# ashawkey/nerf2mesh

Hardware: AMD Instinct MI355X
Metric: train_samples_per_sec (higher is better)
Workload: dtype f32 march/composite, f16 autocast encode+MLP (reference -O recipe); 1 GPU; nerf_synthetic/lego stage-0 -O --bound 1 --dt_gamma 0, 800x800 x 100 synthetic views, num_points target 2^18/GPU (adaptive num_rays), occupancy refresh every 16 steps; diffuse_step=1000, refresh_steps_in_window=64, parallelism=single GPU, occupancy_refresh=single GPU, mlp=fused MFMA field kernels, driver=engine.Stage0Engine (fixed launch sequence), pretrain_steps=1000, params=18367240

## Files before the change

### include/n2m_hip.h

```cpp
#ifndef N2M_HIP_H
#define N2M_HIP_H

#include <stdint.h>

#ifdef __cplusplus
extern "C" {
#endif

#define N2M_ABI_VERSION 1

enum { N2M_F32 = 0, N2M_F16 = 1 };

enum {
    N2M_OK = 0,
    N2M_EINVAL = -1,
    N2M_ENULL = -2,
    N2M_EUNSUPPORTED = -3
};

int n2m_abi_version(void);
const char* n2m_last_error(void);


int n2m_near_far_from_aabb(const float* rays_o, const float* rays_d, const float* aabb, uint32_t N,
// ... 100 lines not shown
                                const int32_t* offsets, void* grad_embeddings, uint32_t B, uint32_t D,
                                uint32_t C, uint32_t L, uint32_t max_level, float S, uint32_t H,
                                uint32_t gridtype, int align_corners, uint32_t interp, int dtype,
                                void* stream);

uint64_t n2m_grid_binned_workspace_bytes(uint32_t B, uint32_t D, uint32_t C, uint32_t max_level,
                                         const int32_t* host_offsets, int dtype, int tv);
int n2m_grid_encode_backward_binned(const void* grad, const float* inputs, const int32_t* host_offsets,
                                    void* grad_embeddings, uint32_t B, uint32_t D, uint32_t C, uint32_t L,
                                    uint32_t max_level, float S, uint32_t H, uint32_t gridtype, int align_corners,
                                    uint32_t interp, int dtype, const float* tv_embeddings, float tv_weight,
                                    float tv_weight_outer, float tv_inner01, const float* tv_scale,
                                    float* found_inf, void* workspace, uint64_t workspace_bytes, void* stream);
int n2m_grad_total_variation_binned(const float* inputs, const float* embeddings, float* grad,
                                    const int32_t* host_offsets, float weight, float weight_outer, float inner01,
                                    const float* weight_scale, uint32_t B, uint32_t D, uint32_t C, uint32_t L, float S,
                                    uint32_t H, uint32_t gridtype, int align_corners, void* workspace,
                                    uint64_t workspace_bytes, void* stream);

int n2m_grid_encode_forward_pair(const float* inputs, const float* embeddings1, const void* embeddings2,
                                 const int32_t* offsets, float* outputs1, void* outputs2, uint32_t B, uint32_t L,
                                 uint32_t max_level, float S, uint32_t H, uint32_t gridtype, int align_corners,
                                 uint32_t interp, float in_scale, float in_offset, void* stream);

int n2m_grid_encode_forward_packed(const float* inputs, const void* packed, const int32_t* offsets, float* outputs1,
                                   void* outputs2, uint32_t B, uint32_t L, uint32_t max_level, float S, uint32_t H,
                                   uint32_t gridtype, int align_corners, uint32_t interp, float in_scale, float in_offset,
                                   void* stream);
int n2m_grid_encode_forward_packed_tv(const float* inputs, const void* packed, const int32_t* offsets, float* outputs1,
                                      void* outputs2, uint32_t B, uint32_t L, uint32_t max_level, float S, uint32_t H,
                                      uint32_t gridtype, int align_corners, uint32_t interp, float in_scale, float in_offset,
                                      float* tv_corners, void* stream);
int n2m_grid_encode_forward_packed_tvterms(const float* inputs, const void* packed, const int32_t* offsets, float* outputs1,
                                           void* outputs2, uint32_t B, uint32_t L, uint32_t max_level, float S, uint32_t H,
                                           uint32_t gridtype, int align_corners, uint32_t interp, float in_scale, float in_offset,
                                           float tv_weight, float tv_weight_outer, float tv_inner01, const float* tv_scale,
                                           float* tv_out, void* stream);
int n2m_grid_backward_tv_corners(const float* tv_corners);

int n2m_grid_encode_forward_packed_levels(const float* inputs, const void* packed, const int32_t* offsets, float* outputs1,
                                          void* outputs2, uint32_t B, uint32_t L, uint32_t max_level, float S, uint32_t H,
                                          uint32_t gridtype, int align_corners, uint32_t interp, float in_scale, float in_offset,
                                          uint32_t level_begin, uint32_t n_levels, void* stream);

uint64_t n2m_grid_binned_pair_workspace_bytes(uint32_t B, uint32_t max_level, const int32_t* host_offsets);
int n2m_grid_encode_backward_binned_pair(const float* grad1, const void* grad2, const float* inputs,
// ... 377 lines not shown
```

### include/n2m_mlp.h

```cpp
#ifndef N2M_MLP_H
#define N2M_MLP_H

#include <stdint.h>

#ifdef __cplusplus
extern "C" {
#endif

int n2m_field_forward(const float* xyz, const float* dirs, const float* h1, const void* h2, const float* w_sigma0,
                      const float* w_sigma1, const float* w_color0, const float* w_color1, const float* w_color2,
                      const float* w_spec0, const float* w_spec1, uint32_t M, int shading, int normalize_dirs, float* sigma, float* rgb,
                      float* specular, void* stream);

int n2m_field_backward(const float* xyz, const float* dirs, const float* h1, const void* h2, const float* w_sigma0,
                       const float* w_sigma1, const float* w_color0, const float* w_color1, const float* w_color2,
                       const float* w_spec0, const float* w_spec1, uint32_t M, int shading, int normalize_dirs, const float* d_sigma,
                       const float* d_rgb, const float* d_specular, float* d_h1, void* d_h2, float* d_w_sigma0,
                       float* d_w_sigma1, float* d_w_color0, float* d_w_color1, float* d_w_color2, float* d_w_spec0,
                       float* d_w_spec1, float* found_inf, void* stream);

int n2m_field_forward_train(const float* xyz, const float* dirs, const float* h1, const void* h2, const float* w_sigma0,
                            const float* w_sigma1, const float* w_color0, const float* w_color1, const float* w_color2,
                            const float* w_spec0, const float* w_spec1, uint32_t M, int shading, int normalize_dirs, float* sigma, float* rgb,
                            float* specular, float* spec_sq_partial, void* stream);
int n2m_field_backward_train(const float* xyz, const float* dirs, const float* h1, const void* h2, const float* w_sigma0,
                             const float* w_sigma1, const float* w_color0, const float* w_color1, const float* w_color2,
                             const float* w_spec0, const float* w_spec1, uint32_t M, int shading, int normalize_dirs, const float* d_sigma,
                             const float* d_rgb, const float* d_specular, float* d_h1, void* d_h2, float* d_w_sigma0,
                             float* d_w_sigma1, float* d_w_color0, float* d_w_color1, float* d_w_color2, float* d_w_spec0,
                             float* d_w_spec1, float* found_inf, float spec_reg, const float* seed, void* stream);
uint32_t n2m_field_spec_partials(void);

#ifdef __cplusplus
}
#endif
// ... 2 lines not shown
```

### nerf2mesh_amd/_lib.py

```python
import ctypes
import os
import threading

_HERE = os.path.dirname(os.path.abspath(__file__))
LIB_PATH = os.environ.get("N2M_HIP_LIB") or os.path.join(_HERE, "lib", "libn2m_hip.so")

_u32, _i32, _f32, _vp, _int, _u64 = ctypes.c_uint32, ctypes.c_int32, ctypes.c_float, ctypes.c_void_p, ctypes.c_int, ctypes.c_uint64

SIGNATURES = {
    "n2m_near_far_from_aabb": [_vp, _vp, _vp, _u32, _f32, _vp, _vp, _vp],
    "n2m_sph_from_ray": [_vp, _vp, _f32, _u32, _vp, _vp],
    "n2m_morton3D": [_vp, _u32, _vp, _vp],
    "n2m_morton3D_invert": [_vp, _u32, _vp, _vp],
    "n2m_packbits": [_vp, _u32, _f32, _vp, _vp],
    "n2m_packbits_dev": [_vp, _u32, _vp, _vp, _vp],
    "n2m_flatten_rays": [_vp, _u32, _u32, _vp, _vp],
    "n2m_march_rays_train": [_vp, _vp, _vp, _f32, _int, _f32, _u32, _u32, _u32, _u32, _vp, _vp, _vp, _vp, _vp, _vp, _vp, _vp, _vp],
    "n2m_march_rays_train_write": [_vp, _vp, _vp, _f32, _int, _f32, _u32, _u32, _u32, _u32, _vp, _vp, _vp, _vp, _vp, _vp, _vp, _u32, _vp],
    "n2m_march_rays_train_fused": [_vp, _vp, _vp, _f32, _int, _f32, _u32, _u32, _u32, _u32, _vp, _vp, _vp, _vp, _vp, _vp, _vp, _vp, _u32, _vp, _u64, _vp],
    "n2m_march_fused_workspace_bytes": [_u32],
    "n2m_march_fallback_count": [_vp],
    "n2m_debug_fill_times": [_int, _vp],
    "n2m_stream_copy": [_vp, _vp, _u64, _u32, _vp],
    "n2m_composite_live_counts": [_vp, _vp],
# ... 5 lines not shown
    "n2m_composite_rays_train_forward": [_vp, _vp, _vp, _vp, _u32, _u32, _f32, _int, _vp, _vp, _vp, _vp, _vp],
    "n2m_composite_rays_train_backward": [_vp, _vp, _vp, _vp, _vp, _vp, _vp, _vp, _vp, _vp, _vp, _u32, _u32, _f32, _int, _vp, _vp, _vp],
    "n2m_composite_loss_train": [_vp, _vp, _vp, _vp, _u32, _u32, _f32, _vp, _vp, _f32, _f32, _f32, _vp, _vp, _vp, _vp, _vp, _vp, _vp, _vp, _vp, _vp],
    "n2m_composite_loss_train_ent": [_vp, _vp, _vp, _vp, _u32, _u32, _f32, _vp, _vp, _f32, _f32, _f32, _vp, _vp, _vp, _vp, _vp, _vp, _vp, _vp, _vp, _f32, _vp],
    "n2m_composite_loss_train_depth": [_vp, _vp, _vp, _vp, _u32, _u32, _f32, _vp, _vp, _f32, _f32, _f32, _vp, _vp, _vp, _vp, _vp, _vp, _vp, _vp, _vp, _f32,
                                       _vp, _vp, _vp, _f32, _int, _vp],
    "n2m_composite_loss_train_ex": [_vp, _vp, _vp, _vp, _u32, _u32, _f32, _vp, _vp, _f32, _f32, _f32, _vp, _vp, _vp, _vp, _vp, _vp, _vp, _vp, _vp, _f32, _int, _vp],
    "n2m_march_rays": [_u32, _u32, _vp, _vp, _vp, _vp, _f32, _int, _f32, _u32, _u32, _u32, _vp, _vp, _vp, _vp, _vp, _vp, _vp, _vp],
    "n2m_composite_rays": [_u32, _u32, _f32, _int, _vp, _vp, _vp, _vp, _vp, _vp, _vp, _vp, _vp],
    "n2m_compact_alive": [_vp, _u32, _vp, _vp, _vp],
    "n2m_select_positive": [_vp, _u32, _u32, _vp, _vp, _vp],
    "n2m_march_rays_dev": [_vp, _u32, _u32, _vp, _vp, _vp, _vp, _f32, _int, _f32, _u32, _u32, _u32, _vp, _vp, _vp, _vp, _vp, _vp, _vp],
    "n2m_composite_rays_dev": [_vp, _u32, _u32, _u32, _f32, _int, _vp, _vp, _vp, _vp, _vp, _vp, _vp, _vp, _vp],
    "n2m_compact_alive_dev": [_vp, _vp, _u32, _u32, _u32, _vp, _vp, _vp],
    "n2m_grid_encode_forward": [_vp, _vp, _vp, _vp, _u32, _u32, _u32, _u32, _u32, _f32, _u32, _vp, _u32, _int, _u32, _int, _vp],
    "n2m_grid_encode_backward": [_vp, _vp, _vp, _vp, _vp, _u32, _u32, _u32, _u32, _u32, _f32, _u32, _vp, _vp, _u32, _int, _u32, _int, _vp],
    "n2m_grad_total_variation": [_vp, _vp, _vp, _vp, _f32, _u32, _u32, _u32, _u32, _f32, _u32, _u32, _int, _int, _vp],
    "n2m_grid_encode_forward_bm": [_vp, _vp, _vp, _vp, _u32, _u32, _u32, _u32, _u32, _f32, _u32, _u32, _int, _u32, _int, _vp],
    "n2m_grid_encode_backward_bm": [_vp, _vp, _vp, _vp, _vp, _u32, _u32, _u32, _u32, _u32, _f32, _u32, _u32, _int, _u32, _int, _vp],
    "n2m_grid_binned_workspace_bytes": [_u32, _u32, _u32, _u32, _vp, _int, _int],
    "n2m_grid_encode_backward_binned": [_vp, _vp, _vp, _vp, _u32, _u32, _u32, _u32, _u32, _f32, _u32, _u32, _int, _u32, _int,
                                        _vp, _f32, _f32, _f32, _vp, _vp, _vp, _u64, _vp],
    "n2m_grid_encode_forward_pair": [_vp, _vp, _vp, _vp, _vp, _vp, _u32, _u32, _u32, _f32, _u32, _u32, _int, _u32, _f32, _f32, _vp],
    "n2m_grid_encode_forward_packed": [_vp, _vp, _vp, _vp, _vp, _u32, _u32, _u32, _f32, _u32, _u32, _int, _u32, _f32, _f32, _vp],
    "n2m_grid_encode_forward_packed_tv": [_vp, _vp, _vp, _vp, _vp, _u32, _u32, _u32, _f32, _u32, _u32, _int, _u32, _f32, _f32, _vp, _vp],
    "n2m_grid_encode_forward_packed_tvterms": [_vp, _vp, _vp, _vp, _vp, _u32, _u32, _u32, _f32, _u32, _u32, _int, _u32, _f32, _f32, _f32, _f32, _f32, _vp, _vp, _vp],
    "n2m_grid_backward_tv_corners": [_vp],
    "n2m_grid_encode_forward_packed_levels": [_vp, _vp, _vp, _vp, _vp, _u32, _u32, _u32, _f32, _u32, _u32, _int, _u32, _f32, _f32, _u32, _u32, _vp],
    "n2m_grid_binned_pair_workspace_bytes": [_u32, _u32, _vp],
    "n2m_grid_encode_backward_binned_pair": [_vp, _vp, _vp, _vp, _vp, _vp, _u32, _u32, _u32, _f32, _u32, _u32, _int, _u32,
                                             _vp, _f32, _f32, _f32, _vp, _vp, _f32, _f32, _int, _vp, _u64, _vp],
    "n2m_grid_encode_backward_binned_pair_half": [_vp, _vp, _vp, _vp, _vp, _vp, _u32, _u32, _u32, _f32, _u32, _u32, _int, _u32,
                                                  _vp, _f32, _f32, _f32, _vp, _vp, _f32, _f32, _int, _vp, _u64, _vp, _int],
    "n2m_sdf_fold_plan": [_vp, _u32, _f32, _f32, _u32, _u32, _f32, _u32, _int, _vp, _vp, _vp, _u32, _vp, _u32, _vp],
    "n2m_sdf_fold_gather": [_vp, _u32, _u32, _vp, _vp, _u32, _vp, _u32, _vp, _vp],
    "n2m_grid_encode_backward_binned_lists": [_vp, _vp, _u32, _vp, _vp, _u32, _u32, _u32, _f32, _u32, _u32, _int, _u32, _vp, _int, _vp, _u64, _vp],
    "n2m_grid_encode_backward_binned_pair_fold": [_vp, _vp, _vp, _vp, _vp, _vp, _u32, _u32, _u32, _f32, _u32, _u32, _int, _u32,
                                                  _vp, _f32, _f32, _f32, _vp, _vp, _f32, _f32, _int, _vp, _u64, _vp, _vp, _f32, _f32, _vp],
    "n2m_occupancy_update_partials": [_u32],
    "n2m_occupancy_points": [_vp, _vp, _vp, _f32, _f32, _vp, _u32, _vp],
    "n2m_occupancy_update": [_vp, _vp, _f32, _u32, _f32, _vp, _vp, _vp, _vp, _vp],
    "n2m_grid_pair_fuse_plan": [_u32, _u32, _vp, ctypes.POINTER(ctypes.c_uint32), ctypes.POINTER(ctypes.c_uint32)],
    "n2m_grid_encode_backward_binned_pair_adam": [_vp, _vp, _vp, _vp, _vp, _vp, _u32, _u32, _u32, _f32, _u32, _u32, _int, _u32,
                                                  _vp, _f32, _f32, _f32, _vp, _vp, _f32, _f32, _vp, _u64, _vp, _vp],
    "n2m_adam_fuse_restore": [_vp, _vp, _u32, _vp, _vp],
    "n2m_grid_tv_terms": [_vp, _vp, _vp, _u32, _u32, _f32, _u32, _u32, _int, _u32, _f32, _f32, _f32, _vp, _f32, _f32, _vp, _vp],
# ... 63 lines not shown
    "n2m_capture_view": [_vp, _u32, _u32, _u32, _u32, _u32, _f32, _f32, _f32, _f32, _vp, _vp, _vp, _vp, _vp, _vp, _u32, _vp],
    "n2m_capture_box_downscale": [_vp, _u32, _u32, _u32, _u32, _vp, _vp],
    "n2m_adam_step": [_vp, ctypes.c_double, ctypes.c_double, _f32, _vp, _vp, _vp, _vp],
    "n2m_adam_step_scaler": [_vp, ctypes.c_double, ctypes.c_double, _f32, _vp, _vp, _vp, _vp, _vp],
    "n2m_ema_update": [_vp, _f32, _vp],
    "n2m_scaler_update": [_vp, _vp, _vp, _vp, _vp, ctypes.c_double, ctypes.c_double, _f32, _f32, _f32, _vp],
    "n2m_scaler_update_slots": [_vp, _vp, _vp, _vp, _vp, _u32, ctypes.c_double, ctypes.c_double, _f32, _f32, _f32, _vp],
    "n2m_scaler_update_slots_loss": [_vp, _vp, _vp, _vp, _vp, _u32, ctypes.c_double, ctypes.c_double, _f32, _f32, _f32, _vp, _u32, _u32, _vp, _vp, _vp],
    "n2m_scaler_update_slots_loss2": [_vp, _vp, _vp, _vp, _vp, _u32, ctypes.c_double, ctypes.c_double, _f32, _f32, _f32, _vp, _u32, _u32, _vp, _vp,
                                      _vp, _u32, _f32, _vp],
    "n2m_scaler_update_slots_loss3": [_vp, _vp, _vp, _vp, _vp, _u32, ctypes.c_double, ctypes.c_double, _f32, _f32, _f32, _vp, _u32, _u32, _vp, _vp,
                                      _vp, _u32, _f32, _vp, _u32, _f32, _vp],
    "n2m_sdf_offsets": [_vp, _u32, _f32, _f32, _vp, _vp, _vp],
    "n2m_sdf_alpha_forward": [_vp, _vp, _vp, _vp, _u32, _vp, _f32, _f32, _vp, _vp, _vp, _vp],
    "n2m_sdf_alpha_backward": [_vp, _vp, _vp, _vp, _vp, _u32, _vp, _f32, _f32, _vp, _f32, _vp, _vp, _vp, _vp, _vp, _vp],
    "n2m_photo_loss_forward": [_vp, _vp, _vp, _vp, _f32, _f32, _f32, _u32, _vp, _vp, _vp, _vp],
    "n2m_photo_loss_backward": [_vp, _vp, _vp, _vp, _f32, _f32, _f32, _u32, _vp, _vp, _vp, _vp],
    "n2m_sh_encode_forward": [_vp, _vp, _u32, _u32, _u32, _vp, _vp],
    "n2m_sh_encode_backward": [_vp, _vp, _u32, _u32, _u32, _vp, _vp, _vp],
    "n2m_field_forward": [_vp] * 11 + [_u32, _int, _int] + [_vp] * 4,
    "n2m_field_backward": [_vp] * 11 + [_u32, _int, _int] + [_vp] * 14,
    "n2m_field_forward_train": [_vp] * 11 + [_u32, _int, _int] + [_vp] * 5,
    "n2m_field_backward_train": [_vp] * 11 + [_u32, _int, _int] + [_vp] * 13 + [_f32, _vp, _vp],
    "n2m_field_spec_partials": [],
    "n2m_rasterize_forward": [_vp, _vp, _u32, _u32, _u32, _u32, _vp, _vp, _vp],
    "n2m_rasterize_backward": [_vp, _vp, _vp, _vp, _u32, _u32, _u32, _u32, _vp, _vp],
    "n2m_interpolate_forward": [_vp, _vp, _vp, _u32, _u32, _u32, _u32, _u32, _vp, _vp],
    "n2m_interpolate_backward": [_vp, _vp, _vp, _vp, _u32, _u32, _u32, _u32, _u32, _vp, _vp, _vp],
    "n2m_interpolate_backward_strided": [_vp, _vp, _vp, _vp, _u32, _u32, _u32, _u32, _u32, _u32, _vp, _vp, _vp],
    "n2m_antialias_build_topology": [_vp, _u32, _vp, _u32, _vp],
    "n2m_antialias_forward": [_vp, _vp, _vp, _vp, _vp, _u32, _u32, _u32, _u32, _u32, _u32, _vp, _vp],
    "n2m_antialias_backward": [_vp, _vp, _vp, _vp, _vp, _u32, _vp, _u32, _u32, _u32, _u32, _u32, _f32, _vp, _vp, _vp],
    "n2m_antialias_backward_seeded": [_vp, _vp, _vp, _vp, _vp, _u32, _vp, _u32, _u32, _u32, _u32, _u32, _f32, _vp, _vp, _vp],
    "n2m_to_clip": [_vp, _vp, _u32, _vp, _vp],
    "n2m_to_clip_backward": [_vp, _vp, _u32, _vp, _vp],
    "n2m_laplacian_forward": [_vp, _vp, _vp, _u32, _vp, _f32, _f32, _f32, _u32, _vp, _vp, _vp, _vp],
    "n2m_laplacian_backward": [_vp, _vp, _vp, _vp, _u32, _vp, _f32, _vp, _f32, _f32, _u32, _vp, _vp, _vp],
    "n2m_laplacian_backward_acc": [_vp, _vp, _vp, _vp, _u32, _vp, _f32, _vp, _f32, _f32, _u32, _vp, _vp, _vp],
    "n2m_mesh_losses_forward": [_vp, _vp, _u32, _vp, _u32, _f32, _f32, _vp, _vp],
    "n2m_mesh_losses_backward": [_vp, _vp, _vp, _vp, _u32, _vp, _vp, _vp, _u32, _u32, _vp, _f32, _f32, _vp, _vp],
    "n2m_mesh_losses_backward_acc": [_vp, _vp, _vp, _vp, _u32, _vp, _vp, _vp, _u32, _u32, _vp, _f32, _f32, _vp, _vp],
    "n2m_gather_rows": [_vp, _vp, _u32, _u32, _vp, _vp],
    "n2m_gather_rows_strided": [_vp, _vp, _u32, _u32, _u32, _vp, _u32, _vp],
    "n2m_scatter_rows_strided": [_vp, _vp, _u32, _u32, _u32, _vp, _u32, _vp],
    "n2m_scatter_rows": [_vp, _vp, _u32, _u32, _vp, _vp],
    "n2m_stage1_head": [_vp, _vp, _vp, _u32, _u32, _u32, _vp, _vp, _f32, _f32, _f32, _vp, _vp, _vp, _vp, _vp, _vp, _vp, _vp, _vp, _vp, _int, _vp, _vp, _vp],
# ... 190 lines not shown
```

### nerf2mesh_amd/csrc/gridencoder.hip

```cpp
#include <math.h>
#include <stdlib.h>

#include <atomic>
#include <type_traits>

#include "n2m_common.hpp"
#include "../../include/n2m_peer.h"

namespace {

constexpr uint32_t kMaxLevels = 32;

struct LevelTable {
    float scale[kMaxLevels];
    uint32_t resolution[kMaxLevels];
};

__host__ LevelTable make_levels(uint32_t L, float S, uint32_t H) {
    LevelTable t;
    for (uint32_t l = 0; l < kMaxLevels; ++l) {
        const float sc = l < L ? exp2f((float)l * S) * (float)H - 1.0f : 0.0f;
        t.scale[l] = sc;
        t.resolution[l] = (uint32_t)ceilf(sc) + 1u;
    }
// ... 325 lines not shown
            const bool odd_row = (rx[q] & 1u) != 0u;
            g[2 * q] = odd_row ? pr[q].hi : pr[q].lo;
            g[2 * q + 1] = x_even ? (odd_row ? pr[q].lo : pr[q].hi) : extra[q];
        }
    } else {
#pragma unroll
        for (uint32_t corner = 0; corner < 8; ++corner) {
            const uint32_t v[D] = {cell[0] + (corner & 1u), cell[1] + ((corner >> 1) & 1u), cell[2] + (corner >> 2)};
            g[corner] = Row<T, C>::load(tab + (size_t)ix.row(v) * C);
        }
    }
    Row<T, C> acc;
#pragma unroll
    for (uint32_t c = 0; c < C; ++c) acc.v[c] = (T)0;
#pragma unroll
    for (uint32_t corner = 0; corner < 8; ++corner) {
        float w = 1.0f;
#pragma unroll
        for (uint32_t d = 0; d < D; ++d) w *= (corner & (1u << d)) ? frac[d] : 1 - frac[d];
#pragma unroll
        for (uint32_t c = 0; c < C; ++c) accum(acc.v[c], w, g[corner].v[c]);
    }
    acc.store(out);
}

template <typename T>
__global__ void zero_levels_kernel(T* __restrict__ outputs, uint32_t B, uint32_t LC, uint32_t first, uint32_t count) {
    const uint64_t t = (uint64_t)blockIdx.x * blockDim.x + threadIdx.x;
    if (t >= (uint64_t)B * count) return;
    const uint32_t b = (uint32_t)(t / count), k = (uint32_t)(t - (uint64_t)b * count);
    outputs[(size_t)b * LC + first + k] = (T)0;
}

__device__ __forceinline__ void atomic_add_row(float* dst, const float* v, uint32_t C) {
    for (uint32_t c = 0; c < C; ++c) unsafeAtomicAdd(dst + c, v[c]);
}

struct TvParams {
    const float* table;
    float weight, weight_outer, inner01;
    const float* scale_ptr;
    uint32_t stride = 1;
    const float* corners = nullptr;
};

__device__ __forceinline__ void tv_weights(const TvParams& tv, float& w_in, float& w_out) {
// ... 3785 lines not shown
    N2M_CHECK_LAUNCH();
    return 0;
}

extern "C" int n2m_grid_encode_forward_pair(const float* inputs, const float* embeddings1, const void* embeddings2, const int32_t* offsets,
                                            float* outputs1, void* outputs2, uint32_t B, uint32_t L, uint32_t max_level, float S, uint32_t H,
                                            uint32_t gridtype, int align_corners, uint32_t interp, float in_scale, float in_offset,
                                            void* stream) {
    const char* fn = "grid_encode_forward_pair";
    if (int rc = check_dims(fn, 3, 2, L, max_level, N2M_F16)) return rc;
    N2M_REQUIRE(inputs && embeddings1 && embeddings2 && offsets && outputs1 && outputs2, N2M_ENULL, "%s: NULL tensor", fn);
    if (B == 0 || max_level == 0) return 0;
    hipStream_t s = (hipStream_t)stream;
    const LevelTable lv = make_levels(L, S, H);
    N2M_PROF(N2M_K_GRID_FWD, s, (double)B * (12.0 + (double)max_level * 8 * (4 + 4) + (double)max_level * (4 + 4)));
    const uint32_t n_tiles = n2m_ceil_div(B, 256);
    grid_forward3_pair_kernel<<<n_tiles * max_level, 256, 0, s>>>(inputs, embeddings1, (const _Float16*)embeddings2, offsets, outputs1,
                                                                 (_Float16*)outputs2, B, max_level, lv, gridtype, align_corners != 0, interp, n_tiles,
                                                                 in_scale, in_offset);
    N2M_CHECK_LAUNCH();
    return 0;
}

static int forward_packed(const float* inputs, const void* packed, const int32_t* offsets, float* outputs1, void* outputs2, uint32_t B, uint32_t L,
                          uint32_t max_level, float S, uint32_t H, uint32_t gridtype, int align_corners, uint32_t interp, float in_scale, float in_offset,
                          void* stream, uint32_t level_begin, uint32_t n_levels, float* tv_corners = nullptr, const TvParams* tvp = nullptr,
                          float* tv_out = nullptr);

extern "C" int n2m_grid_encode_forward_packed(const float* inputs, const void* packed, const int32_t* offsets, float* outputs1, void* outputs2,
                                              uint32_t B, uint32_t L, uint32_t max_level, float S, uint32_t H, uint32_t gridtype,
                                              int align_corners, uint32_t interp, float in_scale, float in_offset, void* stream) {
    return forward_packed(inputs, packed, offsets, outputs1, outputs2, B, L, max_level, S, H, gridtype, align_corners, interp, in_scale, in_offset, stream, 0u,
                          max_level);
}

extern "C" int n2m_grid_encode_forward_packed_levels(const float* inputs, const void* packed, const int32_t* offsets, float* outputs1, void* outputs2,
                                                     uint32_t B, uint32_t L, uint32_t max_level, float S, uint32_t H, uint32_t gridtype,
                                                     int align_corners, uint32_t interp, float in_scale, float in_offset, uint32_t level_begin,
                                                     uint32_t n_levels, void* stream) {
    N2M_REQUIRE(n_levels >= 1 && level_begin + n_levels <= max_level, N2M_EINVAL,
                "grid_encode_forward_packed_levels: levels [%u, %u) outside [0, %u)", level_begin, level_begin + n_levels, max_level);
    return forward_packed(inputs, packed, offsets, outputs1, outputs2, B, L, max_level, S, H, gridtype, align_corners, interp, in_scale, in_offset, stream,
                          level_begin, n_levels);
}

static int forward_packed(const float* inputs, const void* packed, const int32_t* offsets, float* outputs1, void* outputs2, uint32_t B, uint32_t L,
// ... 80 lines not shown
```

### nerf2mesh_amd/csrc/mlp.hip

```cpp
#include <map>
#include <mutex>

#include "n2m_common.hpp"
#include "../../include/n2m_mlp.h"

namespace {

typedef _Float16 h4 __attribute__((ext_vector_type(4)));
typedef float f16x __attribute__((ext_vector_type(16)));

#define MFMA(a, b, c) __builtin_amdgcn_mfma_f32_32x32x8f16((a), (b), (c), 0, 0, 0)
typedef _Float16 h8 __attribute__((ext_vector_type(8)));
#define MFMA16(a, b, c) __builtin_amdgcn_mfma_f32_32x32x16_f16((a), (b), (c), 0, 0, 0)

constexpr int P_S0 = 28, P_S1 = 36, P_C0 = 44, P_C1 = 68, P_C2 = 68, P_P0 = 12, P_P1 = 36;
constexpr int P_S1T = 12, P_S0T = 36, P_C2T = 12, P_C1T = 68, P_C0T = 68, P_P1T = 12, P_P0T = 36;
constexpr int O_S0 = 0;
constexpr int O_S1 = O_S0 + 32 * P_S0;
constexpr int O_C0 = O_S1 + 32 * P_S1;
constexpr int O_C1 = O_C0 + 64 * P_C0;
constexpr int O_C2 = O_C1 + 64 * P_C1;
constexpr int O_P0 = O_C2 + 32 * P_C2;
constexpr int O_P1 = O_P0 + 32 * P_P0;
constexpr int FWD_HALVES = O_P1 + 32 * P_P1;
// ... 374 lines not shown
                if (a.shading == 2) { cr = s0; cg = s1; cb = s2; }
                else {
                    cr = fminf(fmaxf((float)(_Float16)(s0 + q0), 0.f), 1.f);
                    cg = fminf(fmaxf((float)(_Float16)(s1 + q1), 0.f), 1.f);
                    cb = fminf(fmaxf((float)(_Float16)(s2 + q2), 0.f), 1.f);
                }
            }
            if (valid && g == 0 && a.rgb) {
                a.rgb[(size_t)s * 3] = cr; a.rgb[(size_t)s * 3 + 1] = cg; a.rgb[(size_t)s * 3 + 2] = cb;
            }
        }
    }
    if (DO_COLOR && a.spec_sq_partial) {
        __shared__ float spec_wave[4];
        const float w = n2m_wave_sum(spec_sq);
        if (lane == 0) spec_wave[threadIdx.x >> 6] = w;
        __syncthreads();
        if (threadIdx.x == 0) a.spec_sq_partial[blockIdx.x] = ((spec_wave[0] + spec_wave[1]) + spec_wave[2]) + spec_wave[3];
        if (blockIdx.x == 0)
            for (int i = (int)gridDim.x + (int)threadIdx.x; i < kSpecPartials; i += 256) a.spec_sq_partial[i] = 0.f;
    }
}

__device__ __forceinline__ void tile_put(_Float16* tile, int kb, const h4& f, int lane) {
    *reinterpret_cast<h4*>(tile + (lane & 31) * TILE_PITCH + 8 * kb + 4 * (lane >> 5)) = f;
}
__device__ __forceinline__ h4 tile_get(const _Float16* tile, int kq, int fb, int lane) {
    const _Float16* p = tile + (8 * kq + 4 * (lane >> 5)) * TILE_PITCH + 32 * fb + (lane & 31);
    h4 r;
    r[0] = p[0]; r[1] = p[TILE_PITCH]; r[2] = p[2 * TILE_PITCH]; r[3] = p[3 * TILE_PITCH];
    return r;
}
typedef short s4v_t __attribute__((__vector_size__(8)));
__device__ __forceinline__ h4 tile_get_tr(const _Float16* tile, int kq, int fb, int lane) {
    const _Float16* p = tile + (8 * kq + 4 * (lane >> 5) + ((lane & 15) >> 2)) * TILE_PITCH + 32 * fb + 16 * ((lane >> 4) & 1) + 4 * (lane & 3);
    return __builtin_bit_cast(h4, __builtin_amdgcn_ds_read_tr16_b64_v4i16((__attribute__((address_space(3))) s4v_t*)p));
}
template <int MB, int NB, bool TR = false>
__device__ __forceinline__ void dw_tile(f16x (&acc)[MB][NB], const _Float16* tY, const _Float16* tX, int lane) {
    if constexpr (TR) {
        h4 ay[4][MB], bx[4][NB];
#pragma unroll
        for (int kq = 0; kq < 4; ++kq) {
#pragma unroll
            for (int mb = 0; mb < MB; ++mb) ay[kq][mb] = tile_get_tr(tY, kq, mb, lane);
#pragma unroll
// ... 615 lines not shown
    N2M_PROF_K(N2M_K_MLP_FWD, s, (double)M * (12 + 64 + 4 + (color ? 64 + 12 + 12 + 12 : 0)));
    const size_t smem = (size_t)FWD_HALVES * 2;
    if (color && density) N2M_LAUNCH((field_forward_kernel<true, true>), persistent_grid(M) * 2, 256, smem, s, a);
    else if (color) N2M_LAUNCH((field_forward_kernel<false, true>), persistent_grid(M) * 2, 256, smem, s, a);
    else N2M_LAUNCH((field_forward_kernel<true, false>), persistent_grid(M) * 2, 256, smem, s, a);
    N2M_CHECK_LAUNCH();
    return 0;
}

extern "C" int n2m_field_forward(const float* xyz, const float* dirs, const float* h1, const void* h2, const float* w_sigma0,
                                 const float* w_sigma1, const float* w_color0, const float* w_color1, const float* w_color2,
                                 const float* w_spec0, const float* w_spec1, uint32_t M, int shading, int normalize_dirs, float* sigma, float* rgb,
                                 float* specular, void* stream) {
    return field_forward_impl(xyz, dirs, h1, h2, w_sigma0, w_sigma1, w_color0, w_color1, w_color2, w_spec0, w_spec1, M, shading, normalize_dirs,
                              sigma, rgb, specular, nullptr, stream);
}
extern "C" int n2m_field_forward_train(const float* xyz, const float* dirs, const float* h1, const void* h2, const float* w_sigma0,
                                       const float* w_sigma1, const float* w_color0, const float* w_color1, const float* w_color2,
                                       const float* w_spec0, const float* w_spec1, uint32_t M, int shading, int normalize_dirs, float* sigma,
                                       float* rgb, float* specular, float* spec_sq_partial, void* stream) {
    return field_forward_impl(xyz, dirs, h1, h2, w_sigma0, w_sigma1, w_color0, w_color1, w_color2, w_spec0, w_spec1, M, shading, normalize_dirs,
                              sigma, rgb, specular, spec_sq_partial, stream);
}
extern "C" uint32_t n2m_field_spec_partials(void) { return (uint32_t)kSpecPartials; }

static int field_backward_impl(const float* xyz, const float* dirs, const float* h1, const void* h2, const float* w_sigma0,
                                  const float* w_sigma1, const float* w_color0, const float* w_color1, const float* w_color2,
                                  const float* w_spec0, const float* w_spec1, uint32_t M, int shading, int normalize_dirs, const float* d_sigma,
                                  const float* d_rgb, const float* d_specular, float* d_h1, void* d_h2, float* d_w_sigma0,
                                  float* d_w_sigma1, float* d_w_color0, float* d_w_color1, float* d_w_color2, float* d_w_spec0,
                                  float* d_w_spec1, float* found_inf, float spec_reg, const float* seed, void* stream) {
    const float* w[7] = {w_sigma0, w_sigma1, w_color0, w_color1, w_color2, w_spec0, w_spec1};
    float* dw[7] = {d_w_sigma0, d_w_sigma1, d_w_color0, d_w_color1, d_w_color2, d_w_spec0, d_w_spec1};
    const bool density = d_sigma != nullptr;
    if (int rc = check_field("field_backward", xyz, h1, w, density, shading)) return rc;
    if (density) N2M_REQUIRE(d_h1 && dw[0] && dw[1], N2M_ENULL, "field_backward: density gradients are NULL");
    const bool color = d_rgb != nullptr;
    N2M_REQUIRE(density || color, N2M_ENULL, "field_backward: both d_sigma and d_rgb are NULL");
    if (color) {
        N2M_REQUIRE(h2 && d_h2 && w[2] && w[3] && w[4] && dw[2] && dw[3] && dw[4], N2M_ENULL, "field_backward: colour branch tensors are NULL");
        if (shading != 0) N2M_REQUIRE(dirs && w[5] && w[6] && dw[5] && dw[6], N2M_ENULL, "field_backward: specular branch tensors are NULL");
    }
    if (M == 0) return 0;
    static bool attr_set = false;
    if (!attr_set) {
        (void)hipFuncSetAttribute((const void*)field_backward_kernel<true, true>, hipFuncAttributeMaxDynamicSharedMemorySize, BWD_HALVES * 2);
// ... 64 lines not shown
```

### nerf2mesh_amd/network.py

```python
import math
import weakref

import torch
import torch.nn as nn
import torch.nn.functional as F

from .activation import trunc_exp
from .encoding import get_encoder
from .renderer import NeRFRenderer


derived_copy_holders = weakref.WeakSet()


def x_is_cuda(net):
    return net.encoder.embeddings.is_cuda


class MLP(nn.Module):

    def __init__(self, dim_in, dim_out, dim_hidden, num_layers, bias=True):
        super().__init__()
        self.dim_in, self.dim_out, self.dim_hidden, self.num_layers = dim_in, dim_out, dim_hidden, num_layers
        self.net = nn.ModuleList([
            nn.Linear(dim_in if l == 0 else dim_hidden, dim_out if l == num_layers - 1 else dim_hidden, bias=bias)
# ... 47 lines not shown
            self.encoder_color._half_version = -1

    def _can_fuse(self, c=None):
        return bool(getattr(self.opt, "fused_mlp", False)) and c is None and x_is_cuda(self)

    def forward(self, x, d, c=None, shading="full", raw_dirs=False):
        if self._can_fuse(c):
            from .fused import fused_field
            return fused_field(self, x.view(-1, 3), d.view(-1, 3), shading, normalize_dirs=raw_dirs)
        assert not raw_dirs
        sigma = self.density(x)["sigma"]
        color, specular = self.rgb(x, d, c, shading)
        return sigma, color, specular

    def density(self, x):
        if self._can_fuse() and not x.requires_grad:
            from .fused import fused_density
            return {"sigma": fused_density(self, x.reshape(-1, 3)).view(x.shape[:-1])}
        h = self.encoder(x, bound=self.bound, max_level=self.max_level)
        h = self.sigma_net(torch.cat([x, h], dim=-1))
        sigma = h[..., 0].float() if self.opt.sdf else trunc_exp(h[..., 0])
        return {"sigma": sigma}

    def init_double_sphere(self, r1=0.5, r2=1.5, iters=8192, batch_size=8192):
        if not self.opt.sdf:
            return
        opt = torch.optim.Adam(list(self.parameters()), lr=1e-3)
        dev = self.embeddings_device()
        for _ in range(iters):
            xyzs = torch.rand(batch_size, 3, device=dev) * 2 * self.bound - self.bound
            d = torch.norm(xyzs, p=2, dim=-1)
            gt = torch.where(d < (r1 + r2) / 2, d - r1, r2 - d)
            loss = F.mse_loss(self.density(xyzs)["sigma"], gt)
            opt.zero_grad()
            loss.backward()
            opt.step()

    def embeddings_device(self):
        return self.encoder.embeddings.device

    def normal(self, x, epsilon=1e-4):
        M = x.shape[0]
        off = torch.zeros(6, 1, 3, device=x.device, dtype=x.dtype)
        for axis in range(3):
            off[2 * axis, 0, axis] = epsilon
            off[2 * axis + 1, 0, axis] = -epsilon
# ... 32 lines not shown
```

### nerf2mesh_amd/renderer.py

```python
import math

import os

import torch
import torch.nn as nn
import torch.nn.functional as F

from . import raymarching
from . import raster as dr


def safe_normalize(x, eps=1e-20):
    return x / torch.sqrt(torch.clamp(torch.sum(x * x, -1, keepdim=True), min=eps))


class _to_clip(torch.autograd.Function):
    @staticmethod
    def forward(ctx, vertices, mvp):
        from . import _lib as L
        vertices, mvp = vertices.float().contiguous(), mvp.float().contiguous()
        clip = torch.empty(vertices.shape[0], 4, dtype=torch.float32, device=vertices.device)
        L.call("n2m_to_clip", L.ptr(vertices), L.ptr(mvp), vertices.shape[0], L.ptr(clip), L.stream())
        ctx.save_for_backward(mvp)
        return clip
# ... 257 lines not shown
            L.call("n2m_compact_alive_dev", p(alive[cur]), p(state[cur]), ub, N, int(max_steps), p(alive[nxt]), p(state[nxt]), s)
            slot = rnd % (run_ahead + 1)
            host[slot].copy_(state[nxt], non_blocking=True)
            events[slot].record()
            pending.append(slot)
            rnd += 1
        self.last_infer_rounds = rnd

    def _sdf_to_alpha(self, sdf, cos, dt):
        inv_s = torch.exp(self.variance * 10.0).clip(1e-6, 1e6)
        prev_cdf = torch.sigmoid((sdf - cos * dt * 0.5) * inv_s)
        next_cdf = torch.sigmoid((sdf + cos * dt * 0.5) * inv_s)
        return ((prev_cdf - next_cdf + 1e-5) / (prev_cdf + 1e-5)).view(-1).clip(0, 1)

    def _cells(self):
        dev = self.density_bitfield.device
        if self._cell_unit is None or self._cell_unit.device != dev:
            H = self.grid_size
            coords = raymarching.morton3D_invert(torch.arange(H ** 3, dtype=torch.int32, device=dev))
            self._cell_unit = 2 * coords.float() / (H - 1) - 1
        return self._cell_unit

    @torch.no_grad()
    def update_extra_state(self, decay=0.95):
        if self.opt.stage > 0:
            return
        from . import _lib as L
        _p = L.ptr
        cells = self._cells()
        grid = self.density_grid
        dev = grid.device
        st = getattr(self, "_refresh_bufs", None)
        if st is None or st["tmp"].shape != grid.shape or st["tmp"].device != dev:
            n_part = int(L.lib().n2m_occupancy_update_partials(grid.numel()))
            st = self._refresh_bufs = {"tmp": torch.empty_like(grid), "xyz": torch.empty_like(cells),
                                       "partials": torch.empty(n_part, dtype=torch.float32, device=dev),
                                       "ticket": torch.zeros(1, dtype=torch.int32, device=dev),
                                       "mean": torch.zeros(1, dtype=torch.float32, device=dev), "thresh": torch.zeros(1, dtype=torch.float32, device=dev)}
        tmp_grid, xyzs = st["tmp"], st["xyz"]
        key = (grid.data_ptr(), grid._version)
        if st.get("valid_key") != key:
            st["valid_key"] = key
            st["valid"] = []
            for cas in range(self.cascade):
                idx = torch.nonzero(grid[cas] >= 0).reshape(-1)
                st["valid"].append(None if idx.numel() == grid.shape[1] else (idx.to(torch.int32), idx))
        n_cells = cells.shape[0]
        if any(v is not None for v in st["valid"]):
            tmp_grid.fill_(-1.0)
        shard = getattr(self, "refresh_shard", None)
        if shard is not None and shard[1] <= 1:
            shard = None
        if shard is not None:
            from .parallel import all_ranks_hold
            if st.get("summary_key") != key:
                vals = []
                for v in st["valid"]:
                    vals += [-1, 0] if v is None else [int(v[0].numel()), int(v[1].sum())]
                st["summary_key"] = key
                st["summary"] = torch.tensor(vals, dtype=torch.int64, device=dev)
            st["shard_ok"] = all_ranks_hold(st["summary"], shard[1])
            if not st["shard_ok"]:
                shard = None
        for cas in range(self.cascade):
            bound = min(2 ** cas, self.bound)
            hgs = bound / self.grid_size
            idx = st["valid"][cas]
            n = n_cells if idx is None else idx[0].numel()
            u = torch.rand_like(cells)
            if n == 0:
                continue
            lo, m = 0, n
            if shard is not None:
                rank, world = shard
                per = (n + world - 1) // world
                lo = min(n, rank * per)
                m = min(n, lo + per) - lo
            sigmas = None
            if m > 0:
                if idx is not None:
                    L.call("n2m_occupancy_points", _p(cells), _p(u), _p(idx[0][lo:lo + m]), float(bound - hgs), float(hgs), _p(xyzs), m, L.stream())
                else:
                    L.call("n2m_occupancy_points", _p(cells[lo:lo + m]), _p(u[lo:lo + m]), None, float(bound - hgs), float(hgs), _p(xyzs), m, L.stream())
                with torch.autocast(device_type="cuda", dtype=torch.float16, enabled=bool(self.opt.fp16)):
                    sigmas = self.density(xyzs[:m])["sigma"].reshape(-1).detach()
                    if self.opt.sdf:
                        inv_s = torch.exp(self.variance * 10.0).clip(1e-6, 1e6)
                        sigmas = torch.sigmoid(-sigmas * inv_s) * inv_s
                sigmas = sigmas.float()
            if shard is not None:
                import torch.distributed as dist
                gath = st.get("gather")
                if gath is None or gath.numel() < per * world:
# ... 388 lines not shown
```

Before: 466.2 million samples/s.

## Fuse occupancy refresh point generation, grid encode, and density MLP into dedicated kernels

Adds a refresh-specific path for the occupancy grid update. One kernel jitters the cell points and encodes the coarse dense levels in a single pass, and a second encodes the remaining levels into a level-major f16 feature buffer. A dedicated density-only MFMA kernel then writes sigma straight into the temporary grid. This replaces the generic occupancy_points, autocast density() and encoder/MLP launches, cutting launch count, intermediate tensors and Python overhead on each refresh. It is enabled by default through an environment flag, applies only in the single-GPU, all-valid-cells, non-SDF case, and moves the first-layer input to f16.

Result: no change. 469.1 million samples/s, median of 6 (+0.6%).

```diff
diff --git a/include/n2m_hip.h b/include/n2m_hip.h
--- a/include/n2m_hip.h
+++ b/include/n2m_hip.h
@@ -146,6 +146,10 @@
                                  const int32_t* offsets, float* outputs1, void* outputs2, uint32_t B, uint32_t L,
                                  uint32_t max_level, float S, uint32_t H, uint32_t gridtype, int align_corners,
                                  uint32_t interp, float in_scale, float in_offset, void* stream);
+int n2m_grid_encode_forward_refresh(float* points, const float* cells, const float* u, float inner, float half_grid_size,
+                                    const float* embeddings, const int32_t* offsets, const int32_t* host_offsets, void* outputs,
+                                    uint32_t B, uint32_t L, uint32_t max_level, float S, uint32_t H, uint32_t gridtype,
+                                    int align_corners, uint32_t interp, float in_scale, float in_offset, void* stream);
 
 int n2m_grid_encode_forward_packed(const float* inputs, const void* packed, const int32_t* offsets, float* outputs1,
                                    void* outputs2, uint32_t B, uint32_t L, uint32_t max_level, float S, uint32_t H,
diff --git a/include/n2m_mlp.h b/include/n2m_mlp.h
--- a/include/n2m_mlp.h
+++ b/include/n2m_mlp.h
@@ -11,6 +11,9 @@
                       const float* w_sigma1, const float* w_color0, const float* w_color1, const float* w_color2,
                       const float* w_spec0, const float* w_spec1, uint32_t M, int shading, int normalize_dirs, float* sigma, float* rgb,
                       float* specular, void* stream);
+
+int n2m_field_density_half(const float* xyz, const void* h1_half, const float* w_sigma0, const float* w_sigma1, uint32_t M, int raw_density,
+                           float* sigma, void* stream);
 
 int n2m_field_backward(const float* xyz, const float* dirs, const float* h1, const void* h2, const float* w_sigma0,
                        const float* w_sigma1, const float* w_color0, const float* w_color1, const float* w_color2,
diff --git a/nerf2mesh_amd/_lib.py b/nerf2mesh_amd/_lib.py
--- a/nerf2mesh_amd/_lib.py
+++ b/nerf2mesh_amd/_lib.py
@@ -51,6 +51,7 @@
     "n2m_grid_encode_backward_binned": [_vp, _vp, _vp, _vp, _u32, _u32, _u32, _u32, _u32, _f32, _u32, _u32, _int, _u32, _int,
                                         _vp, _f32, _f32, _f32, _vp, _vp, _vp, _u64, _vp],
     "n2m_grid_encode_forward_pair": [_vp, _vp, _vp, _vp, _vp, _vp, _u32, _u32, _u32, _f32, _u32, _u32, _int, _u32, _f32, _f32, _vp],
+    "n2m_grid_encode_forward_refresh": [_vp, _vp, _vp, _f32, _f32, _vp, _vp, _vp, _vp, _u32, _u32, _u32, _f32, _u32, _u32, _int, _u32, _f32, _f32, _vp],
     "n2m_grid_encode_forward_packed": [_vp, _vp, _vp, _vp, _vp, _u32, _u32, _u32, _f32, _u32, _u32, _int, _u32, _f32, _f32, _vp],
     "n2m_grid_encode_forward_packed_tv": [_vp, _vp, _vp, _vp, _vp, _u32, _u32, _u32, _f32, _u32, _u32, _int, _u32, _f32, _f32, _vp, _vp],
     "n2m_grid_encode_forward_packed_tvterms": [_vp, _vp, _vp, _vp, _vp, _u32, _u32, _u32, _f32, _u32, _u32, _int, _u32, _f32, _f32, _f32, _f32, _f32, _vp, _vp, _vp],
@@ -160,6 +161,7 @@
     "n2m_field_backward": [_vp] * 11 + [_u32, _int, _int] + [_vp] * 14,
     "n2m_field_forward_train": [_vp] * 11 + [_u32, _int, _int] + [_vp] * 5,
     "n2m_field_backward_train": [_vp] * 11 + [_u32, _int, _int] + [_vp] * 13 + [_f32, _vp, _vp],
+    "n2m_field_density_half": [_vp, _vp, _vp, _vp, _u32, _int, _vp, _vp],
     "n2m_field_spec_partials": [],
     "n2m_rasterize_forward": [_vp, _vp, _u32, _u32, _u32, _u32, _vp, _vp, _vp],
     "n2m_rasterize_backward": [_vp, _vp, _vp, _vp, _u32, _u32, _u32, _u32, _vp, _vp],
diff --git a/nerf2mesh_amd/csrc/gridencoder.hip b/nerf2mesh_amd/csrc/gridencoder.hip
--- a/nerf2mesh_amd/csrc/gridencoder.hip
+++ b/nerf2mesh_amd/csrc/gridencoder.hip
@@ -371,6 +371,143 @@
         for (uint32_t c = 0; c < C; ++c) accum(acc.v[c], w, g[corner].v[c]);
     }
     acc.store(out);
+}
+
+constexpr uint32_t kRefreshCoarseMax = 8;
+
+__device__ __forceinline__ float corner_sum3(const Row<float, 1> (&g)[8], const float (&frac)[3]) {
+    float acc = 0.0f;
+#pragma unroll
+    for (uint32_t corner = 0; corner < 8; ++corner) {
+        float w = 1.0f;
+#pragma unroll
+        for (uint32_t d = 0; d < 3; ++d) w *= (corner & (1u << d)) ? frac[d] : 1 - frac[d];
+        accum(acc, w, g[corner].v[0]);
+    }
+    return acc;
+}
+
+template <uint32_t NC>
+__global__ void __launch_bounds__(256)
+grid_refresh_coarse_kernel(float* __restrict__ points, const float* __restrict__ cells, const float* __restrict__ u, float inner, float hgs,
+                           const float* __restrict__ table, const int32_t* __restrict__ offsets, _Float16* __restrict__ out, uint32_t B,
+                           LevelTable lv, uint32_t gridtype, uint32_t interp, float in_scale, float in_offset) {
+    constexpr uint32_t D = 3;
+    const uint32_t b = blockIdx.x * 256u + threadIdx.x;
+    if (b >= B) return;
+    float x[D];
+    if (cells) {
+#pragma unroll
+        for (uint32_t d = 0; d < D; ++d) {
+            const float jitter = (u[(size_t)b * D + d] * 2.0f - 1.0f) * hgs;
+            x[d] = cells[(size_t)b * D + d] * inner + jitter;
+            points[(size_t)b * D + d] = x[d];
+        }
+    } else {
+        load_point<D>(points, b, x);
+    }
+    if constexpr (NC > 0) {
+#pragma unroll
+        for (uint32_t d = 0; d < D; ++d) x[d] = x[d] * in_scale + in_offset;
+        if (outside_unit_cube<D>(x)) {
+#pragma unroll
+            for (uint32_t l = 0; l < NC; ++l) out[(size_t)l * B + b] = (_Float16)0;
+            return;
+        }
+        Row<float, 1> g[NC][8];
+        float frac[NC][D];
+#pragma unroll
+        for (uint32_t l = 0; l < NC; ++l) {
+            const uint32_t row0 = (uint32_t)offsets[l];
+            const uint32_t size = (uint32_t)offsets[l + 1] - row0;
+            const Indexer<D> ix(size, lv.resolution[l], gridtype, false);
+            const float* __restrict__ tab = table + (size_t)row0;
+            uint32_t cell[D];
+            float dfrac[D];
+            locate<D>(x, lv.scale[l], false, interp, cell, frac[l], dfrac);
+            const uint32_t base = cell[0] + cell[1] * ix.stride[1] + cell[2] * ix.stride[2];
+#pragma unroll
+            for (uint32_t q = 0; q < 4; ++q) {
+                const uint32_t r = base + ((q & 1u) ? ix.stride[1] : 0u) + ((q & 2u) ? ix.stride[2] : 0u);
+                const RowPair<float, 1> pr = load_pair<float, 1>(tab + (size_t)r);
+                g[l][2 * q] = pr.lo; g[l][2 * q + 1] = pr.hi;
+            }
+        }
+#pragma unroll
+        for (uint32_t l = 0; l < NC; ++l) out[(size_t)l * B + b] = (_Float16)corner_sum3(g[l], frac[l]);
+    }
+}
+
+__global__ void __launch_bounds__(256)
+grid_refresh_levels_kernel(const float* __restrict__ points, const float* __restrict__ table, const int32_t* __restrict__ offsets,
+                           _Float16* __restrict__ out, uint32_t B, uint32_t level_begin, uint32_t max_level, LevelTable lv, uint32_t gridtype,
+                           bool align_corners, uint32_t interp, uint32_t n_tiles, float in_scale, float in_offset) {
+    constexpr uint32_t D = 3;
+    const uint32_t rel = blockIdx.x / n_tiles, tile = blockIdx.x - rel * n_tiles;
+    const uint32_t level = level_begin + rel;
+    if (level >= max_level) return;
+    const uint32_t b = tile * 256u + threadIdx.x;
+    if (b >= B) return;
+    const uint32_t row0 = (uint32_t)offsets[level];
+    const uint32_t size = (uint32_t)offsets[level + 1] - row0;
+    const float scale = lv.scale[level];
+    const Indexer<D> ix(size, lv.resolution[level], gridtype, align_corners);
+    const float* __restrict__ tab = table + (size_t)row0;
+    _Float16* o = out + (size_t)level * B + b;
+
+    float x[D];
+    load_point<D>(points, b, x);
+#pragma unroll
+    for (uint32_t d = 0; d < D; ++d) x[d] = x[d] * in_scale + in_offset;
+    if (outside_unit_cube<D>(x)) {
+        *o = (_Float16)0;
+        return;
+    }
+    uint32_t cell[D];
+    float frac[D], dfrac[D];
+    locate<D>(x, scale, align_corners, interp, cell, frac, dfrac);
+
+    Row<float, 1> g[8];
+    const bool dense = !ix.hashed && !ix.wrap;
+    if (dense) {
+        const uint32_t base = cell[0] + cell[1] * ix.stride[1] + cell[2] * ix.stride[2];
+#pragma unroll
+        for (uint32_t q = 0; q < 4; ++q) {
+            const uint32_t r = base + ((q & 1u) ? ix.stride[1] : 0u) + ((q & 2u) ? ix.stride[2] : 0u);
+            const RowPair<float, 1> pr = load_pair<float, 1>(tab + (size_t)r);
+            g[2 * q] = pr.lo; g[2 * q + 1] = pr.hi;
+        }
+    } else if (ix.hashed && ix.pow2) {
+        const uint32_t hy0 = cell[1] * kPrimes[1], hy1 = hy0 + kPrimes[1], hz0 = cell[2] * kPrimes[2], hz1 = hz0 + kPrimes[2];
+        const bool x_even = (cell[0] & 1u) == 0u;
+        uint32_t rx[4], rx1[4];
+        RowPair<float, 1> pr[4];
+#pragma unroll
+        for (uint32_t q = 0; q < 4; ++q) {
+            const uint32_t h = ((q & 1u) ? hy1 : hy0) ^ ((q & 2u) ? hz1 : hz0);
+            rx[q] = (cell[0] ^ h) & ix.mask;
+            rx1[q] = ((cell[0] + 1u) ^ h) & ix.mask;
+            pr[q] = load_pair<float, 1>(tab + (size_t)(rx[q] & ~1u));
+        }
+        Row<float, 1> extra[4];
+        if (!x_even) {
+#pragma unroll
+            for (uint32_t q = 0; q < 4; ++q) extra[q] = Row<float, 1>::load(tab + (size_t)rx1[q]);
+        }
+#pragma unroll
+        for (uint32_t q = 0; q < 4; ++q) {
+            const bool odd_row = (rx[q] & 1u) != 0u;
+            g[2 * q] = odd_row ? pr[q].hi : pr[q].lo;
+            g[2 * q + 1] = x_even ? (odd_row ? pr[q].lo : pr[q].hi) : extra[q];
+        }
+    } else {
+#pragma unroll
+        for (uint32_t corner = 0; corner < 8; ++corner) {
+            const uint32_t v[D] = {cell[0] + (corner & 1u), cell[1] + ((corner >> 1) & 1u), cell[2] + (corner >> 2)};
+            g[corner] = Row<float, 1>::load(tab + (size_t)ix.row(v));
+        }
+    }
+    *o = (_Float16)corner_sum3(g, frac);
 }
 
 template <typename T>
@@ -4202,6 +4339,53 @@
     return 0;
 }
 
+static bool level_is_dense3(uint32_t size, uint32_t resolution, bool align_corners) {
+    uint32_t s = 1;
+    for (uint32_t d = 0; d < 3; ++d)
+        if (s <= size) s *= align_corners ? resolution : resolution + 1u;
+    return s <= size && !align_corners;
+}
+
+template <uint32_t NC>
+static void launch_refresh_coarse(uint32_t nc, float* points, const float* cells, const float* u, float inner, float hgs, const float* table,
+                                  const int32_t* offsets, _Float16* out, uint32_t B, const LevelTable& lv, uint32_t gridtype, uint32_t interp,
+                                  float in_scale, float in_offset, hipStream_t s) {
+    if (nc == NC) {
+        grid_refresh_coarse_kernel<NC><<<n2m_ceil_div(B, 256), 256, 0, s>>>(points, cells, u, inner, hgs, table, offsets, out, B, lv, gridtype, interp,
+                                                                         in_scale, in_offset);
+        return;
+    }
+    if constexpr (NC > 0) launch_refresh_coarse<NC - 1>(nc, points, cells, u, inner, hgs, table, offsets, out, B, lv, gridtype, interp, in_scale, in_offset, s);
+}
+
+extern "C" int n2m_grid_encode_forward_refresh(float* points, const float* cells, const float* u, float inner, float half_grid_size,
+                                               const float* embeddings, const int32_t* offsets, const int32_t* host_offsets, void* outputs,
+                                               uint32_t B, uint32_t L, uint32_t max_level, float S, uint32_t H, uint32_t gridtype,
+                                               int align_corners, uint32_t interp, float in_scale, float in_offset, void* stream) {
+    const char* fn = "grid_encode_forward_refresh";
+    if (int rc = check_dims(fn, 3, 1, L, max_level, N2M_F32)) return rc;
+    N2M_REQUIRE(points && embeddings && offsets && host_offsets && outputs, N2M_ENULL, "%s: NULL tensor", fn);
+    N2M_REQUIRE((cells == nullptr) == (u == nullptr), N2M_EINVAL, "%s: cells and u go together", fn);
+    if (B == 0) return 0;
+    hipStream_t s = (hipStream_t)stream;
+    const LevelTable lv = make_levels(L, S, H);
+    uint32_t nc = 0;
+    while (nc < max_level && nc < kRefreshCoarseMax && host_offsets[nc + 1] > host_offsets[nc] &&
+           level_is_dense3((uint32_t)(host_offsets[nc + 1] - host_offsets[nc]), lv.resolution[nc], align_corners != 0))
+        ++nc;
+    N2M_PROF(N2M_K_GRID_FWD, s, (double)B * (12.0 + (cells ? 36.0 : 0.0) + (double)max_level * 8 * 4 + (double)max_level * 2));
+    if (nc > 0 || cells)
+        launch_refresh_coarse<kRefreshCoarseMax>(nc, points, cells, u, inner, half_grid_size, embeddings, offsets, (_Float16*)outputs, B, lv, gridtype,
+                                                 interp, in_scale, in_offset, s);
+    if (nc < max_level) {
+        const uint32_t n_tiles = n2m_ceil_div(B, 256);
+        grid_refresh_levels_kernel<<<n_tiles * (max_level - nc), 256, 0, s>>>(points, embeddings, offsets, (_Float16*)outputs, B, nc, max_level, lv,
+                                                                              gridtype, align_corners != 0, interp, n_tiles, in_scale, in_offset);
+    }
+    N2M_CHECK_LAUNCH();
+    return 0;
+}
+
 static int forward_packed(const float* inputs, const void* packed, const int32_t* offsets, float* outputs1, void* outputs2, uint32_t B, uint32_t L,
                           uint32_t max_level, float S, uint32_t H, uint32_t gridtype, int align_corners, uint32_t interp, float in_scale, float in_offset,
                           void* stream, uint32_t level_begin, uint32_t n_levels, float* tv_corners = nullptr, const TvParams* tvp = nullptr,
diff --git a/nerf2mesh_amd/csrc/mlp.hip b/nerf2mesh_amd/csrc/mlp.hip
--- a/nerf2mesh_amd/csrc/mlp.hip
+++ b/nerf2mesh_amd/csrc/mlp.hip
@@ -420,6 +420,62 @@
     }
 }
 
+struct RawDensityTile {
+    uint32_t h[8];
+    float xyz[3];
+};
+__device__ __forceinline__ void fetch_density_tile(const FieldArgs& a, const uint16_t* __restrict__ h1h, uint32_t tile, int n, int g, RawDensityTile& r) {
+    const uint32_t s = tile * 32 + (uint32_t)n;
+    const size_t Mz = a.M;
+#pragma unroll
+    for (int i = 0; i < 8; ++i) r.h[i] = 0u;
+#pragma unroll
+    for (int i = 0; i < 3; ++i) r.xyz[i] = 0.f;
+    if (s >= a.M) return;
+#pragma unroll
+    for (int kb = 0; kb < 2; ++kb)
+#pragma unroll
+        for (int i = 0; i < 4; ++i) r.h[4 * kb + i] = h1h[(size_t)(8 * kb + 4 * g + i) * Mz + s];
+    if (g == 0) {
+#pragma unroll
+        for (int i = 0; i < 3; ++i) r.xyz[i] = a.xyz[(size_t)s * 3 + i];
+    }
+}
+__global__ void __launch_bounds__(256) field_density_half_kernel(FieldArgs a, const uint16_t* __restrict__ h1h) {
+    extern __shared__ __attribute__((aligned(16))) _Float16 lds[];
+    stage_images<256, false, true, false>(lds, a);
+
+    const int lane = threadIdx.x & 63, n = lane & 31, g = lane >> 5;
+    const uint32_t wave = blockIdx.x * 4 + (threadIdx.x >> 6), n_waves = gridDim.x * 4;
+    const uint32_t n_tiles = (a.M + 31) / 32;
+    RawDensityTile nxt;
+    fetch_density_tile(a, h1h, wave, n, g, nxt);
+    for (uint32_t tile = wave; tile < n_tiles; tile += n_waves) {
+        const uint32_t s = tile * 32 + n;
+        const bool valid = s < a.M;
+#pragma unroll
+        for (int i = 0; i < 8; ++i) asm volatile("" : "+v"(nxt.h[i]));
+#pragma unroll
+        for (int i = 0; i < 3; ++i) asm volatile("" : "+v"(nxt.xyz[i]));
+        const RawDensityTile cur = nxt;
+        fetch_density_tile(a, h1h, tile + n_waves, n, g, nxt);
+        h4 b0[3];
+#pragma unroll
+        for (int kb = 0; kb < 2; ++kb) {
+            const u2v_t v = {cur.h[4 * kb] | (cur.h[4 * kb + 1] << 16), cur.h[4 * kb + 2] | (cur.h[4 * kb + 3] << 16)};
+            b0[kb] = __builtin_bit_cast(h4, v);
+        }
+        b0[2] = zero4();
+        b0[2][0] = (_Float16)cur.xyz[0]; b0[2][1] = (_Float16)cur.xyz[1]; b0[2][2] = (_Float16)cur.xyz[2];
+        f16x d = zero16();
+        d = mm_k<3>(lds + O_S0, P_S0, 0, b0, d, lane);
+        const h4 b1[4] = {relu_pack<0>(d), relu_pack<1>(d), relu_pack<2>(d), relu_pack<3>(d)};
+        f16x o = zero16();
+        o = mm_k<4>(lds + O_S1, P_S1, 0, b1, o, lane);
+        if (valid && g == 0) a.sigma[s] = a.raw_density ? (float)(_Float16)o[0] : expf((float)(_Float16)o[0]);
+    }
+}
+
 __device__ __forceinline__ void tile_put(_Float16* tile, int kb, const h4& f, int lane) {
     *reinterpret_cast<h4*>(tile + (lane & 31) * TILE_PITCH + 8 * kb + 4 * (lane >> 5)) = f;
 }
@@ -1081,6 +1137,18 @@
     return field_forward_impl(xyz, dirs, h1, h2, w_sigma0, w_sigma1, w_color0, w_color1, w_color2, w_spec0, w_spec1, M, shading, normalize_dirs,
                               sigma, rgb, specular, spec_sq_partial, stream);
 }
+extern "C" int n2m_field_density_half(const float* xyz, const void* h1_half, const float* w_sigma0, const float* w_sigma1, uint32_t M, int raw_density,
+                                      float* sigma, void* stream) {
+    N2M_REQUIRE(xyz && h1_half && w_sigma0 && w_sigma1 && sigma, N2M_ENULL, "field_density_half: NULL tensor");
+    if (M == 0) return 0;
+    FieldArgs a{};
+    a.xyz = xyz; a.w[0] = w_sigma0; a.w[1] = w_sigma1; a.M = M; a.raw_density = raw_density ? 1 : 0; a.sigma = sigma;
+    hipStream_t s = (hipStream_t)stream;
+    N2M_PROF_K(N2M_K_MLP_FWD, s, (double)M * (12 + 32 + 4));
+    N2M_LAUNCH(field_density_half_kernel, persistent_grid(M) * 2, 256, (size_t)FWD_HALVES * 2, s, a, (const uint16_t*)h1_half);
+    N2M_CHECK_LAUNCH();
+    return 0;
+}
 extern "C" uint32_t n2m_field_spec_partials(void) { return (uint32_t)kSpecPartials; }
 
 static int field_backward_impl(const float* xyz, const float* dirs, const float* h1, const void* h2, const float* w_sigma0,
diff --git a/nerf2mesh_amd/network.py b/nerf2mesh_amd/network.py
--- a/nerf2mesh_amd/network.py
+++ b/nerf2mesh_amd/network.py
@@ -1,6 +1,7 @@
 import math
 import weakref
 
+import numpy as np
 import torch
 import torch.nn as nn
 import torch.nn.functional as F
@@ -94,6 +95,35 @@
         sigma = h[..., 0].float() if self.opt.sdf else trunc_exp(h[..., 0])
         return {"sigma": sigma}
 
+    def refresh_query_ready(self):
+        from .fused import _affine
+        enc = self.encoder
+        emb = getattr(enc, "embeddings", None)
+        return bool(self._can_fuse() and not self.opt.sdf and emb is not None and emb.dtype == torch.float32 and emb.dim() == 2
+                    and emb.shape[1] == 1 and getattr(enc, "num_levels", 0) == 16 and getattr(enc, "input_dim", 3) == 3
+                    and hasattr(enc, "host_offsets") and _affine(float(self.bound)) is not None)
+
+    @torch.no_grad()
+    def refresh_query(self, cells, u, inner, hgs, xyz, feat, out):
+        from . import _lib as L
+        from .fused import _affine
+        from .gridencoder import _host_offsets
+        _p = L.ptr
+        enc = self.encoder
+        n = cells.shape[0]
+        max_level = int(min(self.max_level, enc.num_levels))
+        if max_level < enc.num_levels:
+            feat.zero_()
+        aff = _affine(float(self.bound))
+        emb = enc.embeddings.detach().float().contiguous()
+        ho = _host_offsets(enc)
+        L.call("n2m_grid_encode_forward_refresh", _p(xyz), _p(cells), _p(u), float(inner), float(hgs), _p(emb), _p(enc.offsets), ho.ctypes.data,
+               _p(feat), n, enc.num_levels, max_level, float(np.log2(enc.per_level_scale)), int(enc.base_resolution), enc.gridtype_id,
+               int(bool(enc.align_corners)), enc.interp_id, float(aff[0]), float(aff[1]), L.stream())
+        w0 = self.sigma_net.net[0].weight.detach().float().contiguous()
+        w1 = self.sigma_net.net[1].weight.detach().float().contiguous()
+        L.call("n2m_field_density_half", _p(xyz), _p(feat), _p(w0), _p(w1), n, 0, _p(out), L.stream())
+
     def init_double_sphere(self, r1=0.5, r2=1.5, iters=8192, batch_size=8192):
         if not self.opt.sdf:
             return
diff --git a/nerf2mesh_amd/renderer.py b/nerf2mesh_amd/renderer.py
--- a/nerf2mesh_amd/renderer.py
+++ b/nerf2mesh_amd/renderer.py
@@ -303,9 +303,11 @@
         return self._cell_unit
 
     @torch.no_grad()
-    def update_extra_state(self, decay=0.95):
+    def update_extra_state(self, decay=0.95, fused=None):
         if self.opt.stage > 0:
             return
+        if fused is None:
+            fused = os.environ.get("N2M_REFRESH_FUSED", "1") != "0"
         from . import _lib as L
         _p = L.ptr
         cells = self._cells()
@@ -343,6 +345,11 @@
             st["shard_ok"] = all_ranks_hold(st["summary"], shard[1])
             if not st["shard_ok"]:
                 shard = None
+        fused = bool(fused and shard is None and all(v is None for v in st["valid"]) and cells.is_cuda
+                     and getattr(self, "refresh_query_ready", lambda: False)())
+        self.last_refresh_fused = fused
+        if fused and st.get("feat") is None:
+            st["feat"] = torch.empty(16, n_cells, dtype=torch.float16, device=dev)
         for cas in range(self.cascade):
             bound = min(2 ** cas, self.bound)
             hgs = bound / self.grid_size
@@ -350,6 +357,9 @@
             n = n_cells if idx is None else idx[0].numel()
             u = torch.rand_like(cells)
             if n == 0:
+                continue
+            if fused:
+                self.refresh_query(cells, u, float(bound - hgs), float(hgs), xyzs, st["feat"], tmp_grid[cas])
                 continue
             lo, m = 0, n
             if shard is not None:
```
